# qianlim/CAPE

Measured on AMD Instinct MI355X. Metric: meshes/sec fwd+bwd, CAPE-affineconv nz64 @ batch 16, 1/2/4/8 MI355X, higher is better.
Workload: dtype f32

## Files before the change

### cape_amd/csrc/gconv.hip

```cpp
#include "common.h"
#include "gconv_shared.h"
#include "gemm_plain.h"
#include "gemm_split.h"
#include "gemm_h2.h"
#include "narrow.h"
#include <stdlib.h>

namespace {

constexpr int KC_DEFAULT = 32;

template <int ROWS, int LDA, int KC, typename AT = float>
__device__ __forceinline__ void stage_gather(float *sA, const SrcDev &S, int n, int r0, int Mo,
                                              int c0, int tid) {
    constexpr int QPR = KC / 4;
    constexpr int RP = 256 / QPR;
    const int q = tid % QPR;
    const int rl0 = tid / QPR;
    const int c = c0 + 4 * q;
    const AT *x0 = reinterpret_cast<const AT *>(S.x) + (long long)n * S.xs;
    const AT *xb = x0 + c;
    const int nvalid = S.C - c;
    constexpr int P = ROWS / RP;
    if (!S.rp && S.vec && (nvalid >= 4 || (nvalid > 0 && c + 4 <= S.ldx) || nvalid <= 0)) {
        float4 v[P];
#pragma unroll
        for (int pass = 0; pass < P; ++pass) {
            const int r = r0 + rl0 + RP * pass;
            const int rc = r < Mo ? r : Mo - 1;
            v[pass] = cape_ld4((nvalid > 0 ? xb : x0) + (long long)rc * S.ldx);
        }
#pragma unroll
        for (int pass = 0; pass < P; ++pass) {
            const bool ok = (r0 + rl0 + RP * pass) < Mo;
            float4 o = v[pass];
            o.x = (ok && nvalid > 0) ? o.x : 0.f; o.y = (ok && nvalid > 1) ? o.y : 0.f;
            o.z = (ok && nvalid > 2) ? o.z : 0.f; o.w = (ok && nvalid > 3) ? o.w : 0.f;
            *reinterpret_cast<float4 *>(&sA[(rl0 + RP * pass) * LDA + 4 * q]) = o;
        }
        return;
    }
#pragma unroll
    for (int pass = 0; pass < P; ++pass) {
        const int rl = rl0 + RP * pass;
        const int r = r0 + rl;
        float4 acc = make_float4(0.f, 0.f, 0.f, 0.f);
        if (r < Mo && nvalid > 0) {
            if (S.vec && nvalid >= 4) {
                const int e1 = S.rp[r + 1];
                int e = S.rp[r];
                for (; e + 1 < e1; e += 2) {
                    const float v0 = S.va[e], v1 = S.va[e + 1];
                    const float4 xa = cape_ld4(xb + (long long)S.ci[e] * S.ldx);
                    const float4 xc = cape_ld4(xb + (long long)S.ci[e + 1] * S.ldx);
                    acc.x = fmaf(v0, xa.x, acc.x); acc.y = fmaf(v0, xa.y, acc.y);
                    acc.z = fmaf(v0, xa.z, acc.z); acc.w = fmaf(v0, xa.w, acc.w);
                    acc.x = fmaf(v1, xc.x, acc.x); acc.y = fmaf(v1, xc.y, acc.y);
                    acc.z = fmaf(v1, xc.z, acc.z); acc.w = fmaf(v1, xc.w, acc.w);
                }
                if (e < e1) {
                    const float v0 = S.va[e];
                    const float4 xa = cape_ld4(xb + (long long)S.ci[e] * S.ldx);
                    acc.x = fmaf(v0, xa.x, acc.x); acc.y = fmaf(v0, xa.y, acc.y);
                    acc.z = fmaf(v0, xa.z, acc.z); acc.w = fmaf(v0, xa.w, acc.w);
                }
            } else {
                float a[4] = {0.f, 0.f, 0.f, 0.f};
                if (S.rp) {
                    const int e1 = S.rp[r + 1];
                    for (int e = S.rp[r]; e < e1; ++e) {
                        const float v = S.va[e];
                        const AT *xr = xb + (long long)S.ci[e] * S.ldx;
#pragma unroll
                        for (int u = 0; u < 4; ++u)
                            if (u < nvalid) a[u] = fmaf(v, cape_ld(xr + u), a[u]);
                    }
                } else {
                    const AT *xr = xb + (long long)r * S.ldx;
#pragma unroll
                    for (int u = 0; u < 4; ++u)
                        if (u < nvalid) a[u] = cape_ld(xr + u);
                }
                acc = make_float4(a[0], a[1], a[2], a[3]);
            }
        }
        *reinterpret_cast<float4 *>(&sA[rl * LDA + 4 * q]) = acc;
    }
}
// ... 431 lines not shown
        a3.x += v3.x; a3.y += v3.y; a3.z += v3.z; a3.w += v3.w;
    }
    for (; sp < p.nsplit; ++sp) {
        const float4 v0 = src[(long long)sp * step];
        a0.x += v0.x; a0.y += v0.y; a0.z += v0.z; a0.w += v0.w;
    }
    float4 t;
    t.x = (a0.x + a1.x) + (a2.x + a3.x); t.y = (a0.y + a1.y) + (a2.y + a3.y);
    t.z = (a0.z + a1.z) + (a2.z + a3.z); t.w = (a0.w + a1.w) + (a2.w + a3.w);
    int si = 0;
    while (si + 1 < p.nsrc && i >= p.part_off[si + 1]) ++si;
    const long long loc = i - p.part_off[si];
    const long long c = loc / p.F, f = loc % p.F;
    float4 *dst = reinterpret_cast<float4 *>(p.w[si] + c * p.wrs[si] + f);
    if (p.accumulate) {
        const float4 o = *dst;
        t.x += o.x; t.y += o.y; t.z += o.z; t.w += o.w;
    }
    *dst = t;
}

__global__ __launch_bounds__(256) void dw_reduce_vec_kernel(DwReduceParams p) { dw_reduce_vec_body(p, blockIdx.x); }

struct DwReduceBatch {
    DwReduceParams it[CAPE_MAX_DW_REDUCE_ITEMS];
    int blk_off[CAPE_MAX_DW_REDUCE_ITEMS + 1];
    int vec[CAPE_MAX_DW_REDUCE_ITEMS];
    int n;
};

__global__ __launch_bounds__(256) void dw_reduce_batch_kernel(DwReduceBatch B) {
    int i = 0;
    while (i + 1 < B.n && (int)blockIdx.x >= B.blk_off[i + 1]) ++i;
    const long long b = (long long)blockIdx.x - B.blk_off[i];
    if (B.vec[i]) dw_reduce_vec_body(B.it[i], b);
    else dw_reduce_body(B.it[i], b);
}

inline int fill_src(SrcDev &d, const cape_src_t &s, int es = 4) {
    if (!s.x || s.C <= 0 || s.ldx < s.C) return CAPE_EINVAL;
    if (s.rowptr && (!s.colidx || !s.vals)) return CAPE_EINVAL;
    d.x = s.x; d.xs = s.x_sample_stride; d.ldx = s.ldx; d.C = s.C;
    d.rp = s.rowptr; d.ci = s.colidx; d.va = s.vals;
    d.w = s.w; d.wrs = s.w_rs; d.wcs = s.w_cs;
    d.w2 = s.w2; d.w2rs = s.w2_rs; d.w2cs = s.w2_cs;
    d.vec = ((s.ldx & 3) == 0) && ((s.x_sample_stride & 3) == 0) && ((reinterpret_cast<uintptr_t>(s.x) & (4 * es - 1)) == 0);
    d.wh = d.wl = d.wh2 = d.wl2 = nullptr;
    d.wp = d.wp2 = 0;
    d.rm = nullptr;
    d.rmw = 0;
    return CAPE_OK;
}

inline int fill_h2(GconvParams &p, const cape_h2_t *h2, bool dual, int out_deinterleave) {
    p.wsi = p.wsi2 = nullptr;
    p.rm_out = nullptr;
    p.rm_out_w = 0;
    if (!h2) return CAPE_OK;
    if (h2->rowmax_out) {
        if (out_deinterleave > 1 || h2->rowmax_out_w < (p.F + 31) / 32 || (h2->rowmax_out_w & 3)) return CAPE_EINVAL;
        p.rm_out = h2->rowmax_out;
        p.rm_out_w = h2->rowmax_out_w;
    }
    if (!h2->src) return CAPE_OK;
    p.wsi = h2->wscale_inv;
    p.wsi2 = dual ? h2->w2scale_inv : nullptr;
    for (int i = 0; i < p.nsrc; ++i) {
        const cape_h2_src_t &h = h2->src[i];
        SrcDev &d = p.s[i];
        d.wh = h.w_hi; d.wl = h.w_lo; d.wp = h.w_pitch;
        d.wh2 = d.w2 ? h.w2_hi : nullptr; d.wl2 = d.w2 ? h.w2_lo : nullptr; d.wp2 = h.w2_pitch;
        d.rm = h.rowmax; d.rmw = h.rowmax_w;
    }
    return CAPE_OK;
}

struct DwPlan {
    int ct, ft, ctiles[CAPE_MAX_SRC], ftiles, ntiles, rsplit, rows_per_split, ngroups, samples_per_group;
    int vstart[CAPE_MAX_SRC + 1];
    long long slab;
};

constexpr int DW_SLOTS_SERIAL = 512, DW_SLOTS_PIPELINED = 256;
inline void plan_dw_splits(int N, int Mo, DwPlan &pl, int slots = DW_SLOTS_SERIAL) {
    int S = slots / pl.ntiles;
    if (S < 1) S = 1;
    int ngroups = 1;
    for (int d = 1; d <= N && d <= S; ++d)
        if (N % d == 0) ngroups = d;
    const int maxr = (Mo + 127) / 128;
    int rsplit = S / ngroups;
    if (rsplit > maxr) rsplit = maxr;
    if (rsplit < 1) rsplit = 1;
    int rows = (Mo + rsplit - 1) / rsplit;
    rows = ((rows + 31) / 32) * 32;
    pl.rows_per_split = rows;
    pl.rsplit = (Mo + rows - 1) / rows;
    pl.samples_per_group = N / ngroups;
    pl.ngroups = ngroups;
}

inline void plan_dw(const cape_src_t *srcs, int nsrc, int N, int Mo, int F, DwPlan &pl) {
    int maxC = 0;
    for (int i = 0; i < nsrc; ++i) maxC = srcs[i].C > maxC ? srcs[i].C : maxC;
    pl.ct = (maxC <= 64) ? 64 : 128;
    pl.ft = (F <= 64) ? 64 : 128;
    pl.ftiles = (F + pl.ft - 1) / pl.ft;
    pl.ntiles = 0;
    pl.slab = 0;
    for (int i = 0; i < nsrc; ++i) {
        pl.ctiles[i] = (srcs[i].C + pl.ct - 1) / pl.ct;
        pl.ntiles += pl.ctiles[i] * pl.ftiles;
        pl.slab += (long long)srcs[i].C * F;
    }
    plan_dw_splits(N, Mo, pl);
}

inline void plan_dw_plain(const cape_src_t *srcs, int nsrc, int N, int Mo, int F, bool pack, DwPlan &pl) {
    int sumC = 0, maxC = 0;
    pl.slab = 0;
    for (int i = 0; i < nsrc; ++i) {
        sumC += srcs[i].C;
        maxC = srcs[i].C > maxC ? srcs[i].C : maxC;
        pl.slab += (long long)srcs[i].C * F;
    }
    const int span = pack ? sumC : maxC;
    const int n128 = (span + 127) / 128, n64 = (span + 63) / 64;
    pl.ft = (F <= 32) ? 32 : (F <= 64) ? 64 : 128;
    pl.ct = (pl.ft == 32 || n64 == 2 * n128) ? 128 : 64;
    pl.ftiles = (F + pl.ft - 1) / pl.ft;
    int v = 0;
    for (int i = 0; i < nsrc; ++i) {
        if (!pack) v = (v + pl.ct - 1) / pl.ct * pl.ct;
        pl.vstart[i] = v;
        v += srcs[i].C;
    }
    pl.vstart[nsrc] = v;
    pl.ntiles = ((v + pl.ct - 1) / pl.ct) * pl.ftiles;
    plan_dw_splits(N, Mo, pl);
}

inline bool dw_srcs_plain(const cape_src_t *srcs, int nsrc, int es = 4) {
    for (int i = 0; i < nsrc; ++i)
        if (srcs[i].rowptr || (((srcs[i].C + 3) & ~3) > srcs[i].ldx) || (srcs[i].ldx & 3) || (srcs[i].x_sample_stride & 3) ||
            (reinterpret_cast<uintptr_t>(srcs[i].x) & (4 * es - 1)))
            return false;
    return true;
}


inline bool dw_dz_vec(const float *dz, int64_t dz_sample_stride, int32_t lddz, const float *dz2, int es = 4) {
    return ((lddz & 3) == 0) && ((dz_sample_stride & 3) == 0) && ((reinterpret_cast<uintptr_t>(dz) & (4 * es - 1)) == 0) &&
           (!dz2 || (reinterpret_cast<uintptr_t>(dz2) & (4 * es - 1)) == 0);
}

inline void fill_h2_dw(DwParams &p, const cape_h2_dw_t *h2) {
    p.dzrm = p.dz2rm = nullptr;
    p.dzrmw = p.dz2rmw = 0;
    if (!h2) return;
    for (int i = 0; i < p.nsrc; ++i) { p.s[i].rm = h2->src_rowmax[i]; p.s[i].rmw = h2->src_rowmax_w[i]; }
    p.dzrm = h2->dz_rowmax; p.dzrmw = h2->dz_rowmax_w;
    p.dz2rm = h2->dz2_rowmax; p.dz2rmw = h2->dz2_rowmax_w;
}

inline int choose_dw(const cape_src_t *srcs, int nsrc, const float *dz, int64_t dz_sample_stride, int32_t lddz,
                     const float *dz2, uint32_t dz2_mask, int N, int Mo, int F, DwPlan &pl, bool bf16 = false) {
    static const int dwp_on = getenv("CAPE_DW_PLAIN") ? atoi(getenv("CAPE_DW_PLAIN")) : 1;
    const int es = bf16 ? 2 : 4;
    const bool dzvec = dw_dz_vec(dz, dz_sample_stride, lddz, dz2, es);
    const bool plain = dwp_on && dzvec && (((F + 3) & ~3) <= lddz) && dw_srcs_plain(srcs, nsrc, es);
    if (bf16) {
        bool c4b = true;
        int sumCb = 0;
        for (int i = 0; i < nsrc; ++i) { c4b = c4b && (srcs[i].C & 3) == 0; sumCb += srcs[i].C; }
        if (plain && c4b && (F & 1) == 0) {
            plan_dw(srcs, nsrc, N, Mo, F, pl);
            return 3;
        }
        if (plain && c4b && !(dz2 && dz2_mask) && nsrc > 1 && sumCb <= 128 && F <= 64) {
            plan_dw_plain(srcs, nsrc, N, Mo, F, true, pl);
            return 2;
        }
        plan_dw(srcs, nsrc, N, Mo, F, pl);
        return plain ? 1 : 0;
    }
    int sumC = 0;
    for (int i = 0; i < nsrc; ++i) sumC += srcs[i].C;
    bool c4 = true;
    for (int i = 0; i < nsrc; ++i) c4 = c4 && (srcs[i].C & 3) == 0;
    const bool packed = plain && c4 && !(dz2 && dz2_mask) && nsrc > 1 && sumC <= 128 && F <= 64;
    static const int dws_on = getenv("CAPE_DW_BF16X6") ? atoi(getenv("CAPE_DW_BF16X6")) : CAPE_DW_BF16X6_DEFAULT;
    const bool dw_split = dws_on && plain && !packed && c4 && (F & 1) == 0;
    if (packed) plan_dw_plain(srcs, nsrc, N, Mo, F, true, pl);
    else plan_dw(srcs, nsrc, N, Mo, F, pl);
    return packed ? 2 : dw_split ? 3 : plain ? 1 : 0;
}

struct FwdPlan {
    int family;
    int BM, BN;
    int layout;
};

inline FwdPlan plan_fwd(const GconvParams &p, const cape_src_t *srcs, bool dual, bool bf16 = false) {
    FwdPlan pl;
    static const int gp_on = getenv("CAPE_GEMM_PLAIN") ? atoi(getenv("CAPE_GEMM_PLAIN")) : 1;
    pl.layout = gp_on ? gp_weight_layout(p, dual) : -1;
    if (bf16) {
        bool ok = pl.layout >= 0 && p.F >= 64;
        for (int i = 0; i < p.nsrc && ok; ++i) {
            const long long ws = srcs[i].w_cs > srcs[i].w_rs ? srcs[i].w_cs : srcs[i].w_rs;
            ok = (srcs[i].ldx & 7) == 0 && (srcs[i].x_sample_stride & 7) == 0 && (reinterpret_cast<uintptr_t>(srcs[i].x) & 15) == 0 &&
                 (long long)p.Mo * srcs[i].ldx < (1LL << 31) && (long long)p.F * ws < (1LL << 31) &&
                 srcs[i].C % GS_KC == 0 && srcs[i].C >= GS_KC;
        }
        if (ok) {
            pl.family = 2;
            gs_tile(dual, p.N, p.Mo, p.F, pl.BM, pl.BN);
            return pl;
        }
        pl.layout = -1;
    }
    for (int i = 0; i < p.nsrc && pl.layout >= 0; ++i) {
        const long long ws = srcs[i].w_cs > srcs[i].w_rs ? srcs[i].w_cs : srcs[i].w_rs;
        if ((long long)p.Mo * srcs[i].ldx >= (1LL << 31) || (long long)p.F * ws >= (1LL << 31)) pl.layout = -1;
    }
    if (pl.layout >= 0 && h2_eligible(p, dual)) {
        pl.family = 3;
        pl.layout = 1;
        int ktot = 0;
        for (int i = 0; i < p.nsrc; ++i) ktot += p.s[i].C;
        h2_tile(dual, p.N, p.Mo, p.F, ktot, pl.BM, pl.BN);
        return pl;
    }
    if (pl.layout >= 0) {
        static const int gs_on = getenv("CAPE_GEMM_BF16X6") ? atoi(getenv("CAPE_GEMM_BF16X6")) : CAPE_GEMM_BF16X6_DEFAULT;
        if (gs_on && gs_eligible(p, dual)) {
            pl.family = 2;
            gs_tile(dual, p.N, p.Mo, p.F, pl.BM, pl.BN);
            return pl;
        }
        static const int narrow_on = getenv("CAPE_NARROW") ? atoi(getenv("CAPE_NARROW")) : 1;
        int sumC = 0;
        for (int i = 0; i < p.nsrc; ++i) sumC += p.s[i].C;
        if (narrow_on && !dual && sumC <= NARROW_MAXC && (p.F & 3) == 0 && p.F >= 16 && p.F <= 256 &&
            (long long)p.N * p.Mo < (1LL << 31)) {
            pl.family = 4;
            pl.BM = 256 / narrow_lpr(p.F / 4); pl.BN = p.F;
            return pl;
        }
        pl.family = 1;
        gp_tile(dual, p.F, pl.BM, pl.BN);
        return pl;
    }
    pl.family = 0;
    pl.BN = (p.F <= 32) ? 32 : (p.F <= 64 || dual) ? 64 : 128;
    pl.BM = 128;
    constexpr int bm64_below = 640;
    if (pl.BN == 128 && (long long)p.N * ((p.Mo + 127) / 128) * ((p.F + 127) / 128) < bm64_below) pl.BM = 64;
    return pl;
}

inline int fill_fwd_srcs(GconvParams &p, const cape_src_t *srcs, int nsrc, bool &dual, int es = 4) {
    dual = false;
    for (int i = 0; i < nsrc; ++i) {
        if (!srcs[i].w) return CAPE_EINVAL;
        int rc = fill_src(p.s[i], srcs[i], es);
        if (rc) return rc;
        dual = dual || (srcs[i].w2 != nullptr);
    }
    p.nsrc = nsrc;
    return CAPE_OK;
}

}

namespace {

// ... 61 lines not shown
    if (pl.family == 4) {
        const bool ok = !p.rankR && !p.mask && dK == 1 && !p.rm_out && (ldy & 3) == 0 && (y_sample_stride & 3) == 0 &&
                        (reinterpret_cast<uintptr_t>(y) & 15) == 0 && (!p.bias || (reinterpret_cast<uintptr_t>(p.bias) & 15) == 0);
        if (ok) {
            const int lpr = narrow_lpr(F / 4), RL = 256 / lpr;
            long long blocks = ((long long)N * Mo + 4 * RL - 1) / (4 * RL);
            if (blocks > 1024) blocks = 1024;
            CAPE_LAUNCH(fwd_narrow_in_kernel, dim3((unsigned)blocks), dim3(256), (size_t)NARROW_MAXC * 4 * lpr * sizeof(float),
                        (hipStream_t)stream, p, lpr);
            CAPE_LAUNCH_CHECK();
            return CAPE_OK;
        }
        pl.family = 1;
        gp_tile(dual, p.F, pl.BM, pl.BN);
    }
    p.row_tiles = (Mo + pl.BM - 1) / pl.BM;
    p.col_tiles = (F + pl.BN - 1) / pl.BN;
    dim3 grid((unsigned)(N * p.row_tiles * p.col_tiles));
    hipStream_t st = (hipStream_t)stream;
    if (pl.family == 3) {
        h2_launch(p, dual, pl.BM, pl.BN, grid, st);
    } else if (pl.family == 2) {
        gs_launch(p, dual, pl.BM, pl.layout, bf16, grid, st);
    } else if (pl.family == 1) {
        gp_launch(p, dual, pl.BM, pl.BN, pl.layout, grid, st);
    } else if (bf16) {
        launch_gather_fwd<cape_bf16>(p, pl, dual, grid, st);
    } else {
        launch_gather_fwd<float>(p, pl, dual, grid, st);
    }
    CAPE_LAUNCH_CHECK();
    return CAPE_OK;
}

}

extern "C" int cape_gconv_fwd_plan(const cape_src_t *srcs, int32_t nsrc, int32_t N, int32_t Mo, int32_t F, int32_t plan[4]) {
    return gconv_fwd_plan_impl(srcs, nsrc, N, Mo, F, plan, false);
}

extern "C" int cape_gconv_fwd_plan_bf16(const cape_src_t *srcs, int32_t nsrc, int32_t N, int32_t Mo, int32_t F, int32_t plan[4]) {
    return gconv_fwd_plan_impl(srcs, nsrc, N, Mo, F, plan, true);
}

extern "C" int cape_gconv_fwd(const cape_src_t *srcs, int32_t nsrc, float *y, int64_t y_sample_stride,
                              int32_t ldy, int32_t N, int32_t Mo, int32_t F, const float *bias,
                              int32_t bias_mode, int32_t act, uint32_t *mask_out, const cape_rank_t *rank,
                              int32_t out_deinterleave, void *stream) {
    return gconv_fwd_impl(srcs, nsrc, y, y_sample_stride, ldy, N, Mo, F, bias, bias_mode, act, mask_out, rank, out_deinterleave,
                          stream, false);
}

extern "C" int cape_gconv_fwd_h2(const cape_src_t *srcs, int32_t nsrc, float *y, int64_t y_sample_stride,
                                 int32_t ldy, int32_t N, int32_t Mo, int32_t F, const float *bias,
                                 int32_t bias_mode, int32_t act, uint32_t *mask_out, const cape_rank_t *rank,
                                 int32_t out_deinterleave, const cape_h2_t *h2, void *stream) {
    return gconv_fwd_impl(srcs, nsrc, y, y_sample_stride, ldy, N, Mo, F, bias, bias_mode, act, mask_out, rank, out_deinterleave,
                          stream, false, h2);
}

extern "C" int cape_gconv_fwd_plan_h2(const cape_src_t *srcs, int32_t nsrc, int32_t N, int32_t Mo, int32_t F, const cape_h2_t *h2,
                                      int32_t plan[4]) {
    return gconv_fwd_plan_impl(srcs, nsrc, N, Mo, F, plan, false, h2);
}

extern "C" int cape_gconv_fwd_bf16(const cape_src_t *srcs, int32_t nsrc, void *y, int64_t y_sample_stride,
                                   int32_t ldy, int32_t N, int32_t Mo, int32_t F, const float *bias,
                                   int32_t bias_mode, int32_t act, uint32_t *mask_out, const cape_rank_t *rank,
                                   int32_t out_deinterleave, void *stream) {
    return gconv_fwd_impl(srcs, nsrc, (float *)y, y_sample_stride, ldy, N, Mo, F, bias, bias_mode, act, mask_out, rank,
                          out_deinterleave, stream, true);
}

extern "C" int64_t cape_gconv_dw_workspace_bytes(const cape_src_t *srcs, int32_t nsrc, int32_t N,
                                                 int32_t Mo, int32_t F) {
    if (!srcs || nsrc < 1 || nsrc > CAPE_MAX_SRC || N < 1 || Mo < 1 || F < 1) return CAPE_EINVAL;
    DwPlan pl;
    plan_dw(srcs, nsrc, N, Mo, F, pl);
    long long need = pl.slab * pl.ngroups * pl.rsplit;
    {
        plan_dw_plain(srcs, nsrc, N, Mo, F, true, pl);
        const long long n2 = pl.slab * pl.ngroups * pl.rsplit;
        need = n2 > need ? n2 : need;
    }
    return (int64_t)need * (int64_t)sizeof(float);
}

namespace {
inline bool dw_takes_h2(const cape_src_t *srcs, int nsrc, const float *dz2, uint32_t dz2_mask, int Mo, int lddz, const cape_h2_dw_t *h2) {
    if (!h2) return false;
    DwParams p;
    p.nsrc = nsrc;
    p.dz2_mask = dz2 ? dz2_mask : 0u;
    p.Mo = Mo; p.lddz = lddz;
    for (int i = 0; i < nsrc; ++i) p.s[i].ldx = srcs[i].ldx;
    fill_h2_dw(p, h2);
    return h2_dw_eligible(p);
}
int gconv_dw_plan_impl(const cape_src_t *srcs, int32_t nsrc, const float *dz, int64_t dz_sample_stride,
                       int32_t lddz, const float *dz2, uint32_t dz2_mask, int32_t N, int32_t Mo, int32_t F,
                       int32_t plan[4], bool bf16, const cape_h2_dw_t *h2 = nullptr) {
    if (!srcs || nsrc < 1 || nsrc > CAPE_MAX_SRC || !dz || N < 1 || Mo < 1 || F < 1 || lddz < F || !plan) return CAPE_EINVAL;
    DwPlan pl;
    plan[0] = choose_dw(srcs, nsrc, dz, dz_sample_stride, lddz, dz2, dz2_mask, N, Mo, F, pl, bf16);
    const int nm = dw_narrow_mode(srcs, nsrc, dz, dz_sample_stride, lddz, dz2, dz2_mask, F, plan[0], bf16);
    if (nm) {
        plan[0] = nm;
    } else if (plan[0] == 3 && !bf16 && dw_takes_h2(srcs, nsrc, dz2, dz2_mask, Mo, lddz, h2)) {
        plan[0] = 4;
        plan_dw_splits(N, Mo, pl, DW_SLOTS_PIPELINED);
    }
    plan[1] = pl.ct; plan[2] = pl.ft; plan[3] = pl.ngroups * pl.rsplit;
    return CAPE_OK;
}
struct DwReduceParams;
int gconv_dw_stage_impl(const cape_src_t *srcs, int32_t nsrc, const float *dz,
                        int64_t dz_sample_stride, int32_t lddz, const float *dz2, uint32_t dz2_mask,
                        int32_t N, int32_t Mo, int32_t F, int32_t accumulate, void *workspace,
                        int64_t workspace_bytes, int32_t stage, void *stream, bool bf16,
                        DwReduceParams *batch_rp = nullptr, int *batch_vec = nullptr, int *batch_blocks = nullptr,
                        const cape_h2_dw_t *h2 = nullptr);
}

extern "C" int cape_gconv_dw_plan(const cape_src_t *srcs, int32_t nsrc, const float *dz, int64_t dz_sample_stride,
                                  int32_t lddz, const float *dz2, uint32_t dz2_mask, int32_t N, int32_t Mo, int32_t F,
                                  int32_t plan[4]) {
    return gconv_dw_plan_impl(srcs, nsrc, dz, dz_sample_stride, lddz, dz2, dz2_mask, N, Mo, F, plan, false);
}

extern "C" int cape_gconv_dw_plan_h2(const cape_src_t *srcs, int32_t nsrc, const float *dz, int64_t dz_sample_stride,
                                     int32_t lddz, const float *dz2, uint32_t dz2_mask, int32_t N, int32_t Mo, int32_t F,
                                     const cape_h2_dw_t *h2, int32_t plan[4]) {
    return gconv_dw_plan_impl(srcs, nsrc, dz, dz_sample_stride, lddz, dz2, dz2_mask, N, Mo, F, plan, false, h2);
}

extern "C" int cape_gconv_dw_stage_h2(const cape_src_t *srcs, int32_t nsrc, const float *dz,
                                      int64_t dz_sample_stride, int32_t lddz, const float *dz2, uint32_t dz2_mask,
                                      int32_t N, int32_t Mo, int32_t F, int32_t accumulate, void *workspace,
                                      int64_t workspace_bytes, int32_t stage, const cape_h2_dw_t *h2, void *stream) {
    if (stage > 2) return CAPE_EINVAL;
    return gconv_dw_stage_impl(srcs, nsrc, dz, dz_sample_stride, lddz, dz2, dz2_mask, N, Mo, F, accumulate, workspace,
                               workspace_bytes, stage, stream, false, nullptr, nullptr, nullptr, h2);
}

extern "C" int cape_gconv_dw_plan_bf16(const cape_src_t *srcs, int32_t nsrc, const void *dz, int64_t dz_sample_stride,
                                       int32_t lddz, const void *dz2, uint32_t dz2_mask, int32_t N, int32_t Mo, int32_t F,
                                       int32_t plan[4]) {
    return gconv_dw_plan_impl(srcs, nsrc, (const float *)dz, dz_sample_stride, lddz, (const float *)dz2, dz2_mask, N, Mo, F, plan, true);
}

extern "C" int cape_gconv_dw_bf16(const cape_src_t *srcs, int32_t nsrc, const void *dz,
                                  int64_t dz_sample_stride, int32_t lddz, const void *dz2, uint32_t dz2_mask,
                                  int32_t N, int32_t Mo, int32_t F, int32_t accumulate, void *workspace,
                                  int64_t workspace_bytes, void *stream) {
    return gconv_dw_stage_impl(srcs, nsrc, (const float *)dz, dz_sample_stride, lddz, (const float *)dz2, dz2_mask, N, Mo, F,
                               accumulate, workspace, workspace_bytes, 0, stream, true);
}

extern "C" int cape_gconv_dw_stage_bf16(const cape_src_t *srcs, int32_t nsrc, const void *dz,
                                        int64_t dz_sample_stride, int32_t lddz, const void *dz2, uint32_t dz2_mask,
                                        int32_t N, int32_t Mo, int32_t F, int32_t accumulate, void *workspace,
                                        int64_t workspace_bytes, int32_t stage, void *stream) {
    if (stage > 2) return CAPE_EINVAL;
    return gconv_dw_stage_impl(srcs, nsrc, (const float *)dz, dz_sample_stride, lddz, (const float *)dz2, dz2_mask, N, Mo, F,
                               accumulate, workspace, workspace_bytes, stage, stream, true);
}

extern "C" int cape_gconv_dw(const cape_src_t *srcs, int32_t nsrc, const float *dz,
                             int64_t dz_sample_stride, int32_t lddz, const float *dz2, uint32_t dz2_mask,
                             int32_t N, int32_t Mo, int32_t F, int32_t accumulate, void *workspace,
                             int64_t workspace_bytes, void *stream) {
    return cape_gconv_dw_stage(srcs, nsrc, dz, dz_sample_stride, lddz, dz2, dz2_mask, N, Mo, F, accumulate, workspace,
                               workspace_bytes, 0, stream);
}

extern "C" int cape_gconv_dw_stage(const cape_src_t *srcs, int32_t nsrc, const float *dz,
                                   int64_t dz_sample_stride, int32_t lddz, const float *dz2, uint32_t dz2_mask,
                                   int32_t N, int32_t Mo, int32_t F, int32_t accumulate, void *workspace,
                                   int64_t workspace_bytes, int32_t stage, void *stream) {
    if (stage > 2) return CAPE_EINVAL;
    return gconv_dw_stage_impl(srcs, nsrc, dz, dz_sample_stride, lddz, dz2, dz2_mask, N, Mo, F, accumulate, workspace,
                               workspace_bytes, stage, stream, false);
}

namespace {
int gconv_dw_stage_impl(const cape_src_t *srcs, int32_t nsrc, const float *dz,
                        int64_t dz_sample_stride, int32_t lddz, const float *dz2, uint32_t dz2_mask,
                        int32_t N, int32_t Mo, int32_t F, int32_t accumulate, void *workspace,
                        int64_t workspace_bytes, int32_t stage, void *stream, bool bf16,
                        DwReduceParams *batch_rp, int *batch_vec, int *batch_blocks, const cape_h2_dw_t *h2) {
    if (stage < 0 || stage > 3 || (stage == 3 && (!batch_rp || !batch_vec || !batch_blocks))) return CAPE_EINVAL;
    if (!srcs || nsrc < 1 || nsrc > CAPE_MAX_SRC || !dz || N < 1 || Mo < 1 || F < 1 || lddz < F || !workspace)
        return CAPE_EINVAL;
    if (dz2_mask && !dz2) return CAPE_EINVAL;
    DwPlan pl;
    const int fam = choose_dw(srcs, nsrc, dz, dz_sample_stride, lddz, dz2, dz2_mask, N, Mo, F, pl, bf16);
    const bool packed = fam == 2, plain = fam != 0, dw_split = fam == 3;
    const int narrow = dw_narrow_mode(srcs, nsrc, dz, dz_sample_stride, lddz, dz2, dz2_mask, F, fam, bf16);
    const bool use_h2 = !narrow && !bf16 && dw_split && dw_takes_h2(srcs, nsrc, dz2, dz2_mask, Mo, lddz, h2);
    if (use_h2) plan_dw_splits(N, Mo, pl, DW_SLOTS_PIPELINED);
    const bool dzvec = dw_dz_vec(dz, dz_sample_stride, lddz, dz2, bf16 ? 2 : 4);
    const long long need = pl.slab * pl.ngroups * pl.rsplit * (long long)sizeof(float);
    if (workspace_bytes < need) return CAPE_EWORKSPACE;
    DwParams p;
    DwReduceParams rp;
    p.nsrc = nsrc; rp.nsrc = nsrc;
    int toff = 0;
    long long poff = 0;
    for (int i = 0; i < nsrc; ++i) {
        if (!srcs[i].w) return CAPE_EINVAL;
        int rc = fill_src(p.s[i], srcs[i], bf16 ? 2 : 4);
        if (rc) return rc;
        p.tile_off[i] = toff; p.part_off[i] = poff; rp.part_off[i] = poff;
        toff += packed ? 0 : pl.ctiles[i] * pl.ftiles;
        poff += (long long)srcs[i].C * F;
        p.vstart[i] = packed ? pl.vstart[i] : 0;
        rp.w[i] = const_cast<float *>(srcs[i].w); rp.wrs[i] = srcs[i].w_rs; rp.wcs[i] = srcs[i].w_cs;
    }
    p.tile_off[nsrc] = toff; p.part_off[nsrc] = poff; rp.part_off[nsrc] = poff;
    p.vstart[nsrc] = packed ? pl.vstart[nsrc] : 0;
    p.dz = dz; p.dz2 = dz2; p.dz2_mask = dz2 ? dz2_mask : 0u; p.dzs = dz_sample_stride; p.lddz = lddz;
    p.dzvec = dzvec;
    p.N = N; p.Mo = Mo; p.F = F; p.ftiles = pl.ftiles;
    p.rsplit = pl.rsplit; p.rows_per_split = pl.rows_per_split;
    p.ngroups = pl.ngroups; p.samples_per_group = pl.samples_per_group;
    p.ws = (float *)workspace; p.slab = pl.slab;
    fill_h2_dw(p, bf16 ? nullptr : h2);
    hipStream_t st = (hipStream_t)stream;
    dim3 grid((unsigned)(pl.ntiles * ((pl.ngroups * pl.rsplit + 7) / 8) * 8)), block(256);
    if (stage >= 2) {
    } else if (narrow == 5) {
        CAPE_LAUNCH(dw_narrow_in_kernel, grid, block, 32768, st, p, narrow_lpr(F / 4), pl.ntiles);
    } else if (narrow == 6) {
        int sumC = 0;
        for (int i = 0; i < nsrc; ++i) sumC += srcs[i].C;
        CAPE_LAUNCH(dw_narrow_out_kernel, grid, block, 16384, st, p, narrow_lpr(sumC / 4), pl.ntiles);
    } else if (use_h2) {
        h2_dw_launch(p, pl.ct, pl.ft, grid, st);
    } else if (bf16 && dw_split) {
        if (pl.ct == 64 && pl.ft == 64) CAPE_LAUNCH((dw_split_kernel<64, 64, cape_bf16>), grid, block, 0, st, p);
        else if (pl.ct == 64) CAPE_LAUNCH((dw_split_kernel<64, 128, cape_bf16>), grid, block, 0, st, p);
        else if (pl.ft == 64) CAPE_LAUNCH((dw_split_kernel<128, 64, cape_bf16>), grid, block, 0, st, p);
        else CAPE_LAUNCH((dw_split_kernel<128, 128, cape_bf16>), grid, block, 0, st, p);
    } else if (bf16 && packed) {
        if (pl.ft == 32) CAPE_LAUNCH((dw_packed_kernel<128, 32, 4, 1, cape_bf16>), grid, block, 0, st, p);
        else if (pl.ct == 64 && pl.ft == 64) CAPE_LAUNCH((dw_packed_kernel<64, 64, 2, 2, cape_bf16>), grid, block, 0, st, p);
        else if (pl.ct == 64) CAPE_LAUNCH((dw_packed_kernel<64, 128, 2, 2, cape_bf16>), grid, block, 0, st, p);
        else if (pl.ft == 64) CAPE_LAUNCH((dw_packed_kernel<128, 64, 2, 2, cape_bf16>), grid, block, 0, st, p);
        else CAPE_LAUNCH((dw_packed_kernel<128, 128, 2, 2, cape_bf16>), grid, block, 0, st, p);
    } else if (bf16 && plain) {
        if (pl.ct == 64 && pl.ft == 64) CAPE_LAUNCH((dw_plain_kernel<64, 64, 2, 2, cape_bf16>), grid, block, 0, st, p);
        else if (pl.ct == 64) CAPE_LAUNCH((dw_plain_kernel<64, 128, 2, 2, cape_bf16>), grid, block, 0, st, p);
        else if (pl.ft == 64) CAPE_LAUNCH((dw_plain_kernel<128, 64, 2, 2, cape_bf16>), grid, block, 0, st, p);
        else CAPE_LAUNCH((dw_plain_kernel<128, 128, 2, 2, cape_bf16>), grid, block, 0, st, p);
    } else if (bf16) {
        if (pl.ct == 64 && pl.ft == 64) CAPE_LAUNCH((gconv_dw_kernel<64, 64, cape_bf16>), grid, block, 0, st, p);
        else if (pl.ct == 64) CAPE_LAUNCH((gconv_dw_kernel<64, 128, cape_bf16>), grid, block, 0, st, p);
        else if (pl.ft == 64) CAPE_LAUNCH((gconv_dw_kernel<128, 64, cape_bf16>), grid, block, 0, st, p);
        else CAPE_LAUNCH((gconv_dw_kernel<128, 128, cape_bf16>), grid, block, 0, st, p);
    } else
    if (packed) {
        if (pl.ft == 32) CAPE_LAUNCH((dw_packed_kernel<128, 32, 4, 1>), grid, block, 0, st, p);
        else if (pl.ct == 64 && pl.ft == 64) CAPE_LAUNCH((dw_packed_kernel<64, 64, 2, 2>), grid, block, 0, st, p);
        else if (pl.ct == 64) CAPE_LAUNCH((dw_packed_kernel<64, 128, 2, 2>), grid, block, 0, st, p);
        else if (pl.ft == 64) CAPE_LAUNCH((dw_packed_kernel<128, 64, 2, 2>), grid, block, 0, st, p);
        else CAPE_LAUNCH((dw_packed_kernel<128, 128, 2, 2>), grid, block, 0, st, p);
    } else if (plain && dw_split) {
        if (pl.ct == 64 && pl.ft == 64) CAPE_LAUNCH((dw_split_kernel<64, 64>), grid, block, 0, st, p);
        else if (pl.ct == 64) CAPE_LAUNCH((dw_split_kernel<64, 128>), grid, block, 0, st, p);
        else if (pl.ft == 64) CAPE_LAUNCH((dw_split_kernel<128, 64>), grid, block, 0, st, p);
        else CAPE_LAUNCH((dw_split_kernel<128, 128>), grid, block, 0, st, p);
    } else if (plain) {
        if (pl.ct == 64 && pl.ft == 64) CAPE_LAUNCH((dw_plain_kernel<64, 64, 2, 2>), grid, block, 0, st, p);
        else if (pl.ct == 64) CAPE_LAUNCH((dw_plain_kernel<64, 128, 2, 2>), grid, block, 0, st, p);
        else if (pl.ft == 64) CAPE_LAUNCH((dw_plain_kernel<128, 64, 2, 2>), grid, block, 0, st, p);
        else CAPE_LAUNCH((dw_plain_kernel<128, 128, 2, 2>), grid, block, 0, st, p);
    } else
    if (pl.ct == 64 && pl.ft == 64) CAPE_LAUNCH((gconv_dw_kernel<64, 64>), grid, block, 0, st, p);
    else if (pl.ct == 64) CAPE_LAUNCH((gconv_dw_kernel<64, 128>), grid, block, 0, st, p);
    else if (pl.ft == 64) CAPE_LAUNCH((gconv_dw_kernel<128, 64>), grid, block, 0, st, p);
    else CAPE_LAUNCH((gconv_dw_kernel<128, 128>), grid, block, 0, st, p);
    CAPE_LAUNCH_CHECK();
    if (stage == 1) return CAPE_OK;
    rp.F = F; rp.nsplit = pl.ngroups * pl.rsplit; rp.accumulate = accumulate; rp.ws = (const float *)workspace; rp.slab = pl.slab;
    long long total = poff;
    int rblocks = (int)((total + 15) / 16);
    bool rvec = (F & 3) == 0 && (pl.slab & 3) == 0 && (reinterpret_cast<uintptr_t>(workspace) & 15) == 0 && total >= 262144;
    for (int i = 0; i < nsrc; ++i)
        rvec = rvec && srcs[i].w_cs == 1 && (srcs[i].w_rs & 3) == 0 && (reinterpret_cast<uintptr_t>(srcs[i].w) & 15) == 0;
    if (stage == 3) {
        *batch_rp = rp;
        *batch_vec = rvec ? 1 : 0;
        *batch_blocks = rvec ? (int)((total / 4 + 255) / 256) : rblocks;
        return CAPE_OK;
    }
    if (rvec) CAPE_LAUNCH(dw_reduce_vec_kernel, dim3((unsigned)((total / 4 + 255) / 256)), dim3(256), 0, st, rp);
    else CAPE_LAUNCH(dw_reduce_kernel, dim3(rblocks), dim3(256), 0, st, rp);
    CAPE_LAUNCH_CHECK();
    return CAPE_OK;
}
}

extern "C" int cape_gconv_dw_reduce_batch(const cape_dw_item_t *items, int32_t nitems, void *stream) {
    if (!items || nitems < 1 || nitems > CAPE_MAX_DW_REDUCE_ITEMS) return CAPE_EINVAL;
    DwReduceBatch B;
    B.n = nitems;
    int off = 0;
    for (int i = 0; i < nitems; ++i) {
        const cape_dw_item_t &t = items[i];
        int blocks = 0;
        const int rc = gconv_dw_stage_impl(t.srcs, t.nsrc, (const float *)t.dz, t.dz_sample_stride, t.lddz, (const float *)t.dz2,
                                           t.dz2_mask, t.N, t.Mo, t.F, t.accumulate, t.workspace, t.workspace_bytes, 3, stream,
                                           t.bf16 != 0, &B.it[i], &B.vec[i], &blocks, t.h2);
        if (rc) return rc;
        B.blk_off[i] = off;
        off += blocks;
    }
    B.blk_off[nitems] = off;
    CAPE_LAUNCH(dw_reduce_batch_kernel, dim3((unsigned)off), dim3(256), 0, (hipStream_t)stream, B);
// ... 4 lines not shown
```

### cape_amd/ops.py

```python
import ctypes as C

import numpy as np
import torch

from . import _lib
from ._lib import lib, CapeSrc, check
from .graph import ConvOperators, HostCSR

import os as _os
FUSED_RECURRENCE = int(_os.environ.get("CAPE_FUSED_RECURRENCE", "1"))
CMR_FUSED_TAIL = int(_os.environ.get("CAPE_CMR_FUSED_TAIL", "1"))
MERGED_D_PASS = _os.environ.get("CAPE_MERGED_D_PASS", "auto")


def merged_d_pass(batch):
    if MERGED_D_PASS == "auto":
        return 2 * int(batch) <= 32
    return bool(int(MERGED_D_PASS))
SPMM_ELL = int(_os.environ.get("CAPE_SPMM_ELL", "1"))

_ACT_OF = {"b1leakyrelu": ("leaky", _lib.BIAS_CHANNEL), "b1relu": ("relu", _lib.BIAS_CHANNEL),
           "b1tanh": ("tanh", _lib.BIAS_CHANNEL), "b2relu": ("relu", _lib.BIAS_VERTEX)}


# ... 172 lines not shown
        if e.get("w2") is not None:
            wt2, off2, rs2, cs2 = e["w2"]
            s.w2, s.w2_rs, s.w2_cs = wt2.data_ptr() + 4 * int(off2), int(rs2), int(cs2)
        else:
            s.w2, s.w2_rs, s.w2_cs = None, 0, 0
    return arr


LAUNCH_LOG = None
PLAN_LOG = None
ACT_TRACE = None
L1_SIGN_TRACE = None


def _trace_sign(y, act):
    if ACT_TRACE is not None and act in ("leaky", "relu"):
        ACT_TRACE.append((y.detach() > 0).cpu())


def _trace_mask_bits(mask, F):
    if ACT_TRACE is not None:
        sh = torch.arange(32, device=mask.device, dtype=torch.int32)
        bits = ((mask.unsqueeze(-1) >> sh) & 1).reshape(mask.shape[0], mask.shape[1], -1)[:, :, :F]
        ACT_TRACE.append((bits != 0).cpu())


def _gconv_work(entries, N, Mo, F):
    es = entries[0]["x"].element_size()
    flops, byts = 0, es * N * Mo * F
    seen = set()
    for e in entries:
        Cs = int(e.get("C", e["x"].shape[2]))
        nblk = 2 if e.get("w2") is not None else 1
        flops += 2 * N * Mo * Cs * F * nblk
        csr = e.get("csr")
        if csr is not None and not csr.identity:
            flops += 2 * N * csr.nnz * Cs
            byts += 8 * csr.nnz + 4 * (csr.shape[0] + 1)
        byts += 4 * Cs * F * nblk
        key = e["x"].data_ptr()
        if key not in seen:
            seen.add(key)
            byts += es * N * e["x"].shape[1] * Cs
    return flops, byts


def _dw_work(entries, N, Mo, F, two_dz):
    es = entries[0]["x"].element_size()
    flops, byts = 0, es * N * Mo * F * (2 if two_dz else 1)
    seen = set()
    for e in entries:
        Cs = int(e.get("C", e["x"].shape[2]))
        flops += 2 * N * Mo * Cs * F
        byts += 4 * Cs * F
        key = e["x"].data_ptr()
        if key not in seen:
            seen.add(key)
            byts += es * N * e["x"].shape[1] * Cs
    return flops, byts


def _csr_bytes(csr):
    return 0 if (csr is None or csr.identity) else 8 * csr.nnz + 4 * (csr.shape[0] + 1)


LOG_SPACER_US = int(_os.environ.get("CAPE_LOG_SPACER_US", "80"))


def _log_launch(name, flops, byts, fn):
    if LAUNCH_LOG is None:
        return fn()
    e0, e1 = torch.cuda.Event(enable_timing=True), torch.cuda.Event(enable_timing=True)
    if LOG_SPACER_US:
        lib.cape_spin_us(LOG_SPACER_US, _stream())
    e0.record()
    out = fn()
    e1.record()
    LAUNCH_LOG.append((name, int(flops), int(byts), e0, e1))
    return out


_FWD_FAMILY = {0: "gconv_fwd_kernel", 1: "gemm_plain_kernel", 2: "gemm_split_kernel", 3: "gemm_h2_kernel", 4: "fwd_narrow_in_kernel"}
_DW_FAMILY = {0: "gconv_dw_kernel", 1: "dw_plain_kernel", 2: "dw_packed_kernel", 3: "dw_split_kernel", 4: "dw_h2_kernel",
              5: "dw_narrow_in_kernel", 6: "dw_narrow_out_kernel"}


def fwd_kernel_name(fam, bm, bn, layout, dual, bf16=False):
    waves = "2, 2" if (bm, bn) in ((64, 128), (128, 128), (64, 64)) else "4, 1"
    tf = lambda b: "true" if b else "false"
    at = ", unsigned short" if bf16 else ", float"
    if fam == 4:
        return "fwd_narrow_in_kernel"
    if fam == 3:
        if (bm, bn) == (128, 256) and not dual:
            return "gemm_h2x_kernel<0, 0>"
        return "gemm_h2_kernel<%d, %d, %s>" % (bm, bn, tf(dual))
    if fam == 2:
        return "gemm_split_kernel<%d, %d, %s, %s%s>" % (bm, bn, tf(layout), tf(dual), at)
    if fam == 1:
        return "gemm_plain_kernel<%d, %d, %s, %s, %s>" % (bm, bn, waves, tf(dual), tf(layout))
    return "gconv_fwd_kernel<%d, %d, %s, %s, 32%s>" % (bm, bn, waves, tf(dual), at)


def dw_kernel_name(fam, ct, ft, bf16=False):
    if fam in (5, 6):
        return _DW_FAMILY[fam]
    if fam == 4:
        return "dw_h2_kernel<%d, %d, %s>" % (ct, ft, "true" if (DW_V4 and (ct, ft) == (128, 128)) else "false")
    if fam == 3 or fam == 0:
        return "%s<%d, %d, %s>" % (_DW_FAMILY[fam], ct, ft, "unsigned short" if bf16 else "float")
    waves = "4, 1" if (fam == 2 and ft == 32) else "2, 2"
    return "%s<%d, %d, %s, %s>" % (_DW_FAMILY[fam], ct, ft, waves, "unsigned short" if bf16 else "float")


FUSE_ACT_GRAD = int(_os.environ.get("CAPE_FUSE_ACT_GRAD", "1"))
FUSE_PREP_SPMM = int(_os.environ.get("CAPE_FUSE_PREP_SPMM", "1"))
DW_V4 = int(_os.environ.get("CAPE_DW_V4", "1"))
_CHAIN = [False]


class _ActOffer(object):
    __slots__ = ("act", "gB", "fused")

    def __init__(self, act, gB):
        self.act, self.gB, self.fused = act, gB, False


class sole_consumer_chain(object):
    def __init__(self, on=True):
        self.on = bool(on)

    def __enter__(self):
        self.prev, _CHAIN[0] = _CHAIN[0], self.on
        return self

    def __exit__(self, *exc):
        _CHAIN[0] = self.prev
        return False


H2 = int(_os.environ.get("CAPE_H2", "1"))
RM_TRACE = int(_os.environ.get("CAPE_RM_TRACE", "0"))


def rm_width(F):
    return ((int(F) + 31) // 32 + 3) // 4 * 4


def alloc_rm(t, F=None):
    return torch.empty((t.shape[0], t.shape[1], rm_width(t.shape[2] if F is None else F)), device=t.device, dtype=torch.float32)


def set_rm(t, rm):
    if rm is not None:
        t._cape_rm = rm
        t._cape_rm_version = t._version
    return t


def drop_rm(t):
    if getattr(t, "_cape_rm", None) is not None:
        t._cape_rm = None


def rm_of(t):
    rm = getattr(t, "_cape_rm", None)
    if rm is None or rm.shape[0] != t.shape[0] or rm.shape[1] != t.shape[1] or rm.device != t.device:
        return None
    if getattr(t, "_cape_rm_version", None) != t._version:
        return None
    return rm


def h2_shape_ok(ktot, F):
    return F >= 64 and (ktot >= 256 or (ktot >= 128 and F >= 128))


def _want_rm(t, Cn=None, any_width=False):
    Cn = t.shape[2] if Cn is None else Cn
    if not (bool(H2) and t.dtype == torch.float32 and Cn % 32 == 0 and Cn >= 32):
        return False
    return any_width or (Cn & (Cn - 1)) == 0


def _new_rm(t):
    return torch.empty((t.shape[0], t.shape[1], 4), device=t.device, dtype=torch.float32)


def rowmax(t):
# ... 2041 lines not shown
```

Baseline: 6509.

## Add thin weight-gradient kernel for packed multi-source small-channel convolutions

Adds a new dw_thin_kernel that computes weight gradients for the packed-family case (one tile, F>32) with 32x32x2 f32 MFMAs. It keeps a three-deep register prefetch pipeline of input and dz loads and reduces the per-wave partial sums through shared memory. Work is split over 256 slots instead of the serial plan, and the workspace query now sizes for this split. The aim is to replace the packed dw kernel with one better suited to thin channel counts. The cost is high register pressure from 8 accumulators of 16 floats each, and an extra shared-memory reduction step.

New measurement: 6563, median of 6. About the same (+0.8%).

```diff
diff --git a/cape_amd/csrc/gconv.hip b/cape_amd/csrc/gconv.hip
--- a/cape_amd/csrc/gconv.hip
+++ b/cape_amd/csrc/gconv.hip
@@ -4,6 +4,7 @@
 #include "gemm_split.h"
 #include "gemm_h2.h"
 #include "narrow.h"
+#include "thin.h"
 #include <stdlib.h>
 
 namespace {
@@ -601,6 +602,9 @@
 };
 
 constexpr int DW_SLOTS_SERIAL = 512, DW_SLOTS_PIPELINED = 256;
+#ifndef CAPE_DW_THIN_SLOTS
+#define CAPE_DW_THIN_SLOTS 256
+#endif
 inline void plan_dw_splits(int N, int Mo, DwPlan &pl, int slots = DW_SLOTS_SERIAL) {
     int S = slots / pl.ntiles;
     if (S < 1) S = 1;
@@ -713,6 +717,22 @@
     if (packed) plan_dw_plain(srcs, nsrc, N, Mo, F, true, pl);
     else plan_dw(srcs, nsrc, N, Mo, F, pl);
     return packed ? 2 : dw_split ? 3 : plain ? 1 : 0;
+}
+
+inline bool thin_on() {
+    static const int on = getenv("CAPE_THIN") ? atoi(getenv("CAPE_THIN")) : 1;
+    return on != 0;
+}
+
+inline bool dw_takes_thin(int fam, int narrow, bool bf16, int N, int Mo, int F, DwPlan &pl) {
+    if (fam != 2 || narrow || bf16 || !thin_on() || pl.ntiles != 1 || F <= 32) return false;
+    plan_dw_splits(N, Mo, pl, CAPE_DW_THIN_SLOTS);
+    const int rows = pl.rows_per_split < Mo ? pl.rows_per_split : Mo;
+    if ((long long)pl.samples_per_group * rows > THIN_MAX_ROWS) {
+        plan_dw_splits(N, Mo, pl);
+        return false;
+    }
+    return true;
 }
 
 struct FwdPlan {
@@ -940,6 +960,9 @@
         plan_dw_plain(srcs, nsrc, N, Mo, F, true, pl);
         const long long n2 = pl.slab * pl.ngroups * pl.rsplit;
         need = n2 > need ? n2 : need;
+        plan_dw_splits(N, Mo, pl, CAPE_DW_THIN_SLOTS);
+        const long long n3 = pl.slab * pl.ngroups * pl.rsplit;
+        need = n3 > need ? n3 : need;
     }
     return (int64_t)need * (int64_t)sizeof(float);
 }
@@ -964,6 +987,10 @@
     const int nm = dw_narrow_mode(srcs, nsrc, dz, dz_sample_stride, lddz, dz2, dz2_mask, F, plan[0], bf16);
     if (nm) {
         plan[0] = nm;
+    } else if (dw_takes_thin(plan[0], nm, bf16, N, Mo, F, pl)) {
+        plan[0] = 7;
+        pl.ct = THIN_MAXV;
+        pl.ft = 64;
     } else if (plan[0] == 3 && !bf16 && dw_takes_h2(srcs, nsrc, dz2, dz2_mask, Mo, lddz, h2)) {
         plan[0] = 4;
         plan_dw_splits(N, Mo, pl, DW_SLOTS_PIPELINED);
@@ -1057,6 +1084,7 @@
     const int narrow = dw_narrow_mode(srcs, nsrc, dz, dz_sample_stride, lddz, dz2, dz2_mask, F, fam, bf16);
     const bool use_h2 = !narrow && !bf16 && dw_split && dw_takes_h2(srcs, nsrc, dz2, dz2_mask, Mo, lddz, h2);
     if (use_h2) plan_dw_splits(N, Mo, pl, DW_SLOTS_PIPELINED);
+    const bool thin = dw_takes_thin(fam, narrow, bf16, N, Mo, F, pl);
     const bool dzvec = dw_dz_vec(dz, dz_sample_stride, lddz, dz2, bf16 ? 2 : 4);
     const long long need = pl.slab * pl.ngroups * pl.rsplit * (long long)sizeof(float);
     if (workspace_bytes < need) return CAPE_EWORKSPACE;
@@ -1093,6 +1121,8 @@
         int sumC = 0;
         for (int i = 0; i < nsrc; ++i) sumC += srcs[i].C;
         CAPE_LAUNCH(dw_narrow_out_kernel, grid, block, 16384, st, p, narrow_lpr(sumC / 4), pl.ntiles);
+    } else if (thin) {
+        CAPE_LAUNCH((dw_thin_kernel<2>), grid, block, 0, st, p);
     } else if (use_h2) {
         h2_dw_launch(p, pl.ct, pl.ft, grid, st);
     } else if (bf16 && dw_split) {
diff --git a/cape_amd/csrc/thin.h b/cape_amd/csrc/thin.h
--- /dev/null
+++ b/cape_amd/csrc/thin.h
@@ -0,0 +1,153 @@
+#pragma once
+#include "common.h"
+#include "gconv_shared.h"
+
+namespace {
+
+constexpr int THIN_DEPTH = 3;
+#define THIN_PIN() do { asm volatile("" ::: "memory"); __builtin_amdgcn_sched_barrier(0); } while (0)
+constexpr int THIN_MAXV = 128;
+constexpr int THIN_MAX_ROWS = 1024;
+
+__device__ __forceinline__ void thin_locate(const DwParams &p, int v, int &si, int &c) {
+    si = 0; c = v;
+#pragma unroll
+    for (int i = 1; i < CAPE_MAX_SRC; ++i)
+        if (i < p.nsrc && v >= p.vstart[i]) { si = i; c = v - p.vstart[i]; }
+}
+
+template <int TN>
+__global__ __launch_bounds__(256, 2) void dw_thin_kernel(DwParams p) {
+    constexpr int D = THIN_DEPTH;
+    __shared__ float red[2 * 4 * 16 * 64];
+    const int tid = threadIdx.x;
+    const int lane = tid & 63, wave = tid >> 6;
+    const int li = lane & 31, lh = lane >> 5;
+
+    const int split = blockIdx.x;
+    if (split >= p.ngroups * p.rsplit) return;
+    const int grp = split / p.rsplit, rs = split % p.rsplit;
+    const int n_begin = grp * p.samples_per_group;
+    const int n_end = min(p.N, n_begin + p.samples_per_group);
+    const int ra = rs * p.rows_per_split;
+    const int rb = min(p.Mo, ra + p.rows_per_split);
+    const int V = p.vstart[p.nsrc];
+
+    const float *xp;
+    long long xs;
+    int ldx;
+    {
+        int si, c;
+        thin_locate(p, 4 * li < V ? 4 * li : 0, si, c);
+        xp = p.s[0].x; xs = p.s[0].xs; ldx = p.s[0].ldx;
+#pragma unroll
+        for (int i = 1; i < CAPE_MAX_SRC; ++i)
+            if (i == si) { xp = p.s[i].x; xs = p.s[i].xs; ldx = p.s[i].ldx; }
+        xp += c;
+    }
+    int fc[TN];
+#pragma unroll
+    for (int b = 0; b < TN; ++b) fc[b] = (b * 32 + li) < p.F ? b * 32 + li : 0;
+
+    f32x16 acc[4][TN];
+#pragma unroll
+    for (int t = 0; t < 4; ++t)
+#pragma unroll
+        for (int b = 0; b < TN; ++b)
+#pragma unroll
+            for (int g = 0; g < 16; ++g) acc[t][b][g] = 0.f;
+
+    const int steps = (rb - ra + 31) / 32;
+    const int total = (n_end - n_begin) * steps;
+
+    if (total > 0) {
+        float4 av[D][4];
+        float bv[D][4][TN];
+        unsigned ok[D];
+        int l_n = n_begin, l_s = 0;
+
+        auto issue = [&](int d) {
+            const int n = l_n < n_end ? l_n : n_end - 1;
+            const float *xb = xp + (long long)n * xs;
+            const float *zb = p.dz + (long long)n * p.dzs;
+            unsigned o = 0;
+#pragma unroll
+            for (int u = 0; u < 4; ++u) {
+                const int r = ra + 32 * l_s + 8 * wave + 2 * u + lh;
+                const int rc = r < rb ? r : rb - 1;
+                o |= ((r < rb && l_n < n_end) ? 1u : 0u) << u;
+                av[d][u] = cape_ld4(xb + (long long)rc * ldx);
+#pragma unroll
+                for (int b = 0; b < TN; ++b) bv[d][u][b] = zb[(long long)rc * p.lddz + fc[b]];
+            }
+            ok[d] = o;
+            if (++l_s == steps) { l_s = 0; ++l_n; }
+        };
+        auto consume = [&](int d) {
+#pragma unroll
+            for (int u = 0; u < 4; ++u) {
+                const bool k = (ok[d] >> u) & 1u;
+                const float a0 = k ? av[d][u].x : 0.f, a1 = k ? av[d][u].y : 0.f;
+                const float a2 = k ? av[d][u].z : 0.f, a3 = k ? av[d][u].w : 0.f;
+#pragma unroll
+                for (int b = 0; b < TN; ++b) {
+                    const float z = k ? bv[d][u][b] : 0.f;
+                    acc[0][b] = __builtin_amdgcn_mfma_f32_32x32x2f32(a0, z, acc[0][b], 0, 0, 0);
+                    acc[1][b] = __builtin_amdgcn_mfma_f32_32x32x2f32(a1, z, acc[1][b], 0, 0, 0);
+                    acc[2][b] = __builtin_amdgcn_mfma_f32_32x32x2f32(a2, z, acc[2][b], 0, 0, 0);
+                    acc[3][b] = __builtin_amdgcn_mfma_f32_32x32x2f32(a3, z, acc[3][b], 0, 0, 0);
+                }
+            }
+        };
+
+#pragma unroll
+        for (int d = 0; d < D; ++d) issue(d);
+        THIN_PIN();
+        for (int it = 0; it < total; it += D) {
+#pragma unroll
+            for (int d = 0; d < D; ++d) {
+                consume(d);
+                THIN_PIN();
+                issue(d);
+                THIN_PIN();
+            }
+        }
+    }
+
+    int ooff[4];
+#pragma unroll
+    for (int j = 0; j < 4; ++j) {
+        const int g = wave + 4 * j;
+        const int v = 4 * ((g & 3) + 8 * (g >> 2) + 4 * lh);
+        int si, c;
+        thin_locate(p, v < V ? v : 0, si, c);
+        long long off = p.part_off[0];
+#pragma unroll
+        for (int i = 1; i < CAPE_MAX_SRC; ++i)
+            if (i == si) off = p.part_off[i];
+        ooff[j] = v < V ? (int)off + c * p.F + li : -1;
+    }
+    const int F = p.F;
+    float *out = p.ws + (long long)split * p.slab;
+#pragma unroll
+    for (int q = 0; q < 2 * TN; ++q) {
+        const int t0 = 2 * (q / TN), b = q % TN;
+        __syncthreads();
+#pragma unroll
+        for (int h = 0; h < 2; ++h)
+#pragma unroll
+            for (int g = 0; g < 16; ++g) red[h * 4096 + (wave * 16 + g) * 64 + lane] = acc[t0 + h][b][g];
+        __syncthreads();
+        const int f = b * 32 + li;
+#pragma unroll
+        for (int h = 0; h < 2; ++h)
+#pragma unroll
+            for (int j = 0; j < 4; ++j) {
+                const int e = h * 4096 + tid + 256 * j;
+                const float sum = (red[e] + red[1024 + e]) + (red[2048 + e] + red[3072 + e]);
+                if (ooff[j] >= 0 && f < F) out[ooff[j] + (t0 + h) * F + b * 32] = sum;
+            }
+    }
+}
+
+}
diff --git a/cape_amd/ops.py b/cape_amd/ops.py
--- a/cape_amd/ops.py
+++ b/cape_amd/ops.py
@@ -278,7 +278,7 @@
 
 _FWD_FAMILY = {0: "gconv_fwd_kernel", 1: "gemm_plain_kernel", 2: "gemm_split_kernel", 3: "gemm_h2_kernel", 4: "fwd_narrow_in_kernel"}
 _DW_FAMILY = {0: "gconv_dw_kernel", 1: "dw_plain_kernel", 2: "dw_packed_kernel", 3: "dw_split_kernel", 4: "dw_h2_kernel",
-              5: "dw_narrow_in_kernel", 6: "dw_narrow_out_kernel"}
+              5: "dw_narrow_in_kernel", 6: "dw_narrow_out_kernel", 7: "dw_thin_kernel"}
 
 
 def fwd_kernel_name(fam, bm, bn, layout, dual, bf16=False):
@@ -301,6 +301,8 @@
 def dw_kernel_name(fam, ct, ft, bf16=False):
     if fam in (5, 6):
         return _DW_FAMILY[fam]
+    if fam == 7:
+        return "dw_thin_kernel<%d>" % (ft // 32)
     if fam == 4:
         return "dw_h2_kernel<%d, %d, %s>" % (ct, ft, "true" if (DW_V4 and (ct, ft) == (128, 128)) else "false")
     if fam == 3 or fam == 0:
```
